# ORNL-Fusion/RAYS

Measured on AMD Instinct MI355X. Metric: ray-steps/sec (whole node), 64k-ray Solovev fan, higher is better.
Workload: dtype f64

## Files before the change

### rays_amd/csrc/rays_device_arith.inc

```
RAYS_DEV double sq(double x) { return x * x; }
RAYS_DEV double pow4(double x) { return ((x * x) * x) * x; }

constexpr int kEqUnitExp = 4;
constexpr int kEqMultiSpec = 8;
constexpr int kEqTol = 16;
constexpr int kEqNoTraj = 32;
constexpr int kEqDeposit = 64;
template <bool MULTI, int NS, int NV>
struct RayVec {
  static constexpr bool DAMP = MULTI || NV == 8 || NV == 13;
  static constexpr int NV0 = 7 + (DAMP ? 1 : 0) + (MULTI ? NS : 0);
  static constexpr bool GRAD = NV == NV0 + 5;
  static_assert(NV == NV0 || NV == NV0 + 5, "nv does not match the damping / gradient options");
};
template <bool UE, bool Y1>
RAYS_DEV double pow_u(double x, double y) {
  if (UE) return Y1 ? x : 1.0;
  if (y == 1.0) return x;
  if (y == 0.0) return 1.0;
  return libm::pow(x, y);
}

struct Recip {
  double d, rc;
// ... 535 lines not shown
    return;
  }
#endif
  const double* const grid = table == 0 ? P.a_rb_grid : (table == 1 ? P.a_ne_grid : (table == 2 ? P.a_te_grid : P.a_ti_grid));
  const double* const fspl = table == 0 ? P.a_rb_fspl : (table == 1 ? P.a_ne_fspl : (table == 2 ? P.a_te_fspl : P.a_ti_fspl));
  spl1_ax<const double*>(grid, fspl, n, P.a_axis[kAxRb + table], x, f, fp);
}

RAYS_DEV void spl1_tab_profiles(const DevParams& P, double psiN, double f[3], double fp[3]) {
  const int n[3] = {P.a_n_ne, P.a_n_te, P.a_n_ti};
#ifndef RAYS_HOST_EMUL
  if (P.a_lds_tab) {
    const eq_lds_ptr base = (eq_lds_ptr)(unsigned long long)P.a_lds_tab;
    const eq_lds_ptr grid[3] = {base + P.a_tab_off[2], base + P.a_tab_off[4], base + P.a_tab_off[6]};
    const eq_lds_ptr fspl[3] = {base + P.a_tab_off[3], base + P.a_tab_off[5], base + P.a_tab_off[7]};
    spl1_ax3<eq_lds_ptr>(grid, fspl, n, &P.a_axis[kAxNe], P.a_profiles_one_grid, psiN, f, fp);
    return;
  }
#endif
  const double* const grid[3] = {P.a_ne_grid, P.a_te_grid, P.a_ti_grid};
  const double* const fspl[3] = {P.a_ne_fspl, P.a_te_fspl, P.a_ti_fspl};
  spl1_ax3<const double*>(grid, fspl, n, &P.a_axis[kAxNe], P.a_profiles_one_grid, psiN, f, fp);
}

RAYS_DEV double eqlin_psi_at(const DevParams& P, int i, int j) {
  long long k = (long long)(i - 1) + (long long)(j - 1) * P.a_nr;
  const long long n = (long long)P.a_nr * P.a_nz;
  k = k < 0 ? 0 : (k >= n ? n - 1 : k);
  return P.a_psi_fspl[k];
}
RAYS_DEV double eqlin_getpsi(const DevParams& P, double R, double Z) {
  const double r1 = P.a_r_grid[0], z1 = P.a_z_grid[0];
  const Recip Rhr = make_recip(P.a_r_grid[1] - r1), Rhz = make_recip(P.a_z_grid[1] - z1);
  const int i = 1 + (int)div(R - r1, Rhr);
  const int j = 1 + (int)div(Z - z1, Rhz);
  const int ic = i < 1 ? 1 : (i > P.a_nr ? P.a_nr : i), jc = j < 1 ? 1 : (j > P.a_nz ? P.a_nz : j);
  const double x = div(R - P.a_r_grid[ic - 1], Rhr);
  const double y = div(Z - P.a_z_grid[jc - 1], Rhz);
  const double omx = 1. - x, omy = 1. - y;
  return ((eqlin_psi_at(P, i, j) * omx * omy + eqlin_psi_at(P, i + 1, j) * x * omy) + eqlin_psi_at(P, i, j + 1) * omx * y) +
         eqlin_psi_at(P, i + 1, j + 1) * x * y;
}
RAYS_DEV double eqlin_getrbphi(const DevParams& P, double R) {
  const double r1 = P.a_r_grid[0];
  const Recip Rhr = make_recip(P.a_r_grid[1] - r1);
  const int i = 1 + (int)div(R - r1, Rhr);
  const int ic = i < 1 ? 1 : (i > P.a_nr - 1 ? P.a_nr - 1 : i);
  const double x = div(R - P.a_r_grid[ic - 1], Rhr);
  return P.a_rb_fspl[ic - 1] * (1. - x) + P.a_rb_fspl[ic] * x;
}
RAYS_DEV void eqlin_psi_grad(const DevParams& P, double R, double Z, double& psi, double& PsiR, double& PsiZ) {
  const double dR = P.a_lin_dR, dZ = P.a_lin_dZ;
  psi = eqlin_getpsi(P, R, Z);
  PsiR = (eqlin_getpsi(P, R + dR, Z) - eqlin_getpsi(P, R - dR, Z)) / 2. / dR;
  PsiZ = (eqlin_getpsi(P, R, Z + dZ) - eqlin_getpsi(P, R, Z - dZ)) / 2. / dZ;
}
RAYS_DEV void eqlin_magnetics(const DevParams& P, double x, double y, double z, double r, const Recip& Rr, double bvec[3],
                              double gbt[3][3], double& psiN, double gradpsiN[3]) {
  const double dR = P.a_lin_dR, dZ = P.a_lin_dZ;
  double psi, PsiR, PsiZ;
  eqlin_psi_grad(P, r, z, psi, PsiR, PsiZ);
  const Recip Rr2 = recip_of_square(sq(r), Rr);
  const Recip RpsiB = const_recip(P.a_psiB, P.a_inv_psiB);
  const double br = div(-PsiZ, Rr);
  const double bz = div(PsiR, Rr);
  const double bphi = div(eqlin_getrbphi(P, r), Rr);
  const double gradpsi[3] = {x * bz, y * bz, -r * br};
  psiN = div(psi, RpsiB);
  gradpsiN[0] = div(gradpsi[0], RpsiB);
  gradpsiN[1] = div(gradpsi[1], RpsiB);
  gradpsiN[2] = div(gradpsi[2], RpsiB);
  const double PsiRZ = (((eqlin_getpsi(P, r + dR, z + dZ) - eqlin_getpsi(P, r - dR, z + dZ)) - eqlin_getpsi(P, r + dR, z - dZ)) +
                        eqlin_getpsi(P, r - dR, z - dZ)) / 4. / dR / dZ;
  const double PsiZZ = ((eqlin_getpsi(P, r, z + 2. * dZ) - 2. * psi) + eqlin_getpsi(P, r, z - 2. * dZ)) / dZ / dZ;
  const double PsiRR = ((eqlin_getpsi(P, r + 2. * dR, z) - 2. * psi) + eqlin_getpsi(P, r - 2. * dR, z)) / dR / dR;
  const double RBphiR = (eqlin_getrbphi(P, r + dR) - eqlin_getrbphi(P, r - dR)) / 2. / dR;
  const double br_r = div(br, Rr), bphi_r = div(bphi, Rr);
  const double dbrdr = -br_r - div(PsiRZ, Rr);
  const double dbrdz = div(-PsiZZ, Rr);
  const double dbzdr = div(-bz, Rr) + div(PsiRR, Rr);
  const double dbzdz = div(PsiRZ, Rr);
  const double dbphidr = div(RBphiR - bphi, Rr);
  bvec[0] = div(br * x, Rr) - div(bphi * y, Rr);
  bvec[1] = div(br * y, Rr) + div(bphi * x, Rr);
  bvec[2] = bz;
  const double x2 = sq(x), y2 = sq(y);
  gbt[0][0] = div(dbrdr * x2 + div(br * y2, Rr) + (-dbphidr + bphi_r) * x * y, Rr2);
  gbt[1][0] = div((dbrdr - br_r) * x * y - dbphidr * y2 - div(bphi * x2, Rr), Rr2);
  gbt[2][0] = div(dbrdz * x, Rr);
  gbt[0][1] = div((dbrdr - br_r) * x * y + dbphidr * x2 + div(bphi * y2, Rr), Rr2);
  gbt[1][1] = div(dbrdr * y2 + div(br * x2, Rr) + (dbphidr - bphi_r) * x * y, Rr2);
  gbt[2][1] = div(dbrdz * y, Rr);
  gbt[0][2] = div(dbzdr * x, Rr);
  gbt[1][2] = div(dbzdr * y, Rr);
  gbt[2][2] = dbzdz;
}

template <int NS, bool UE>
RAYS_DEV int axisym_fields(const DevParams& P, const double rvec[3], double bvec[3], double gbt[3][3],
                           double ns[NS], double gradns[NS][3], double ts[NS], double gradts[NS][3],
                           bool check_box) {
  constexpr double Tiny = 10.0e-14;
  int err = 0;
  const double x = rvec[0], y = rvec[1], z = rvec[2];
  Recip Rr;
  const double r = fsqrt_recip(x * x + y * y, Rr);
  if (r < P.a_box_rmin - Tiny || r > P.a_box_rmax + Tiny) err = RAYS_STOP_AXI_R_OUT_OF_BOX;
  if (z < P.a_box_zmin - Tiny || z > P.a_box_zmax + Tiny) err = RAYS_STOP_AXI_Z_OUT_OF_BOX;
  bool boxed = check_box && err != 0;
  double psiN, gpN[3];
  if (P.a_mag_model == RAYS_AXI_MAG_SOLOVEV) {
    int merr = 0;
    if (r < P.box_rmin || r > P.box_rmax) merr = RAYS_STOP_SOLMAG_R_OUT_OF_BOUNDS;
    if (z < P.box_zmin || z > P.box_zmax) merr = RAYS_STOP_SOLMAG_Z_OUT_OF_BOUNDS;
    if (check_box && !boxed && merr != 0) {
      boxed = true;
      err = merr;
    }
    solovev_magnetics(P, x, y, z, r, Rr, bvec, gbt, psiN, gpN);
  } else if (P.a_mag_model == RAYS_AXI_MAG_EQDSK_LIN) {
    eqlin_magnetics(P, x, y, z, r, Rr, bvec, gbt, psiN, gpN);
  } else {
    double f6[6], RBphi, RBphiR;
    spl2_fpp(P, r, z, f6);
    const double psi = f6[0], PsiR = f6[1], PsiZ = f6[2], PsiRR = f6[3], PsiRZ = f6[4], PsiZZ = f6[5];
    spl1_tab(P, 0, r, RBphi, RBphiR);
    const Recip Rr2 = recip_of_square(sq(r), Rr);
    const Recip RpsiB = const_recip(P.a_psiB, P.a_inv_psiB);
    const double br = div(PsiZ, Rr), bz = div(-PsiR, Rr), bphi = div(RBphi, Rr);
    const double gradpsi[3] = {-x * bz, -y * bz, r * br};
    psiN = div(psi, RpsiB);
    gpN[0] = div(gradpsi[0], RpsiB);
    gpN[1] = div(gradpsi[1], RpsiB);
    gpN[2] = div(gradpsi[2], RpsiB);
    const double br_r = div(br, Rr), bphi_r = div(bphi, Rr);
    const double dbrdr = -br_r + div(PsiRZ, Rr);
    const double dbrdz = div(PsiZZ, Rr);
    const double dbzdr = div(-bz, Rr) - div(PsiRR, Rr);
    const double dbzdz = div(-PsiRZ, Rr);
    const double dbphidr = div(RBphiR - bphi, Rr);
    bvec[0] = div(br * x, Rr) - div(bphi * y, Rr);
    bvec[1] = div(br * y, Rr) + div(bphi * x, Rr);
    bvec[2] = bz;
    const double x2 = sq(x), y2 = sq(y);
    gbt[0][0] = div(dbrdr * x2 + div(br * y2, Rr) + (-dbphidr + bphi_r) * x * y, Rr2);
    gbt[1][0] = div((dbrdr - br_r) * x * y - dbphidr * y2 - div(bphi * x2, Rr), Rr2);
    gbt[2][0] = div(dbrdz * x, Rr);
    gbt[0][1] = div((dbrdr - br_r) * x * y + dbphidr * x2 + div(bphi * y2, Rr), Rr2);
    gbt[1][1] = div(dbrdr * y2 + div(br * x2, Rr) + (dbphidr - bphi_r) * x * y, Rr2);
    gbt[2][1] = div(dbrdz * y, Rr);
    gbt[0][2] = div(dbzdr * x, Rr);
    gbt[1][2] = div(dbzdr * y, Rr);
    gbt[2][2] = dbzdz;
  }
  if (!boxed) err = 0;
  if (!boxed && psiN > P.a_psi_limit) err = RAYS_STOP_OUT_OF_PLASMA;

  bool t_spline = false;
#pragma unroll
  for (int is = 0; is < NS; is++) t_spline = t_spline || P.a_t_model[is] == RAYS_AXI_T_SPLINE;
  const bool batched = t_spline && P.a_n_model == RAYS_AXI_N_SPLINE && P.a_n_ne > 1 && P.a_n_te > 1 && P.a_n_ti > 1;
  double prof[3] = {0., 0., 0.}, dprof[3] = {0., 0., 0.};
  if (batched) spl1_tab_profiles(P, psiN, prof, dprof);

  if (P.a_n_model == RAYS_AXI_N_CONSTANT) {
#pragma unroll
    for (int is = 0; is < NS; is++) {
      ns[is] = P.n0s[is];
      gradns[is][0] = gradns[is][1] = gradns[is][2] = 0.;
    }
  } else {
    double dens = 0., dd_psi = 0.;
    if (P.a_n_model == RAYS_AXI_N_PARABOLIC) {
      parabolic_prof<UE>(psiN, P.a_d_scrape, P.a_an1, P.a_an2, dens, dd_psi);
    } else {
      {
        double d = prof[0], dp = dprof[0];
        if (!batched) spl1_tab(P, 1, psiN, d, dp);
        if (psiN <= 1.0) {
          dens = d;
          dd_psi = dp;
        }
      }
      if (dens < P.a_d_scrape) {
        dens = P.a_d_scrape;
        dd_psi = 0.;
      }
    }
#pragma unroll
    for (int is = 0; is < NS; is++) {
      ns[is] = P.n0s[is] * dens;
      const double c = P.n0s[is] * dd_psi;
      gradns[is][0] = c * gpN[0];
      gradns[is][1] = c * gpN[1];
      gradns[is][2] = c * gpN[2];
    }
  }
#pragma unroll
  for (int is = 0; is < NS; is++) {
    ts[is] = 0.;
    gradts[is][0] = gradts[is][1] = gradts[is][2] = 0.;
  }
#pragma unroll
  for (int is = 0; is < NS; is++) {
    const int m = P.a_t_model[is];
    if (m == RAYS_AXI_T_CONSTANT) {
      ts[is] = P.t0s[is];
#pragma unroll
      for (int j = 0; j < NS; j++) gradts[j][0] = gradts[j][1] = gradts[j][2] = 0.;
    } else if (m == RAYS_AXI_T_PARABOLIC) {
      double t_prof, dt_dpsi;
      parabolic_prof<UE>(psiN, P.a_T_scrape, P.a_at1[is], P.a_at2[is], t_prof, dt_dpsi);
      ts[is] = P.t0s[is] * t_prof;
      const double c = P.t0s[is] * dt_dpsi;
      gradts[is][0] = c * gpN[0];
      gradts[is][1] = c * gpN[1];
      gradts[is][2] = c * gpN[2];
    } else if (m == RAYS_AXI_T_SPLINE) {
      double Te = 0., dTe = 0., Ti = 0., dTi = 0.;
      {
        double te = prof[1], dte = dprof[1], ti = prof[2], dti = dprof[2];
        if (!batched) {
          spl1_tab(P, 2, psiN, te, dte);
          spl1_tab(P, 3, psiN, ti, dti);
        }
        if (psiN <= 1.0) {
          Te = te, dTe = dte, Ti = ti, dTi = dti;
        }
      }
      if (Te < P.a_T_scrape) { Te = P.a_T_scrape; dTe = 0.; }
      if (Ti < P.a_T_scrape) { Ti = P.a_T_scrape; dTi = 0.; }
      const double T = is == 0 ? Te : Ti, dT = is == 0 ? dTe : dTi;
      ts[is] = P.t0s[is] * T;
      const double c = P.t0s[is] * dT;
      gradts[is][0] = c * gpN[0];
      gradts[is][1] = c * gpN[1];
      gradts[is][2] = c * gpN[2];
    }
  }
  if (check_box && !boxed) {
    double mn = ns[0], mt = ts[0];
#pragma unroll
    for (int is = 1; is < NS; is++) {
      if (ns[is] < mn) mn = ns[is];
      if (ts[is] < mt) mt = ts[is];
    }
    if (mn < 0.) err = RAYS_STOP_NEGATIVE_DENS;
    if (mt < 0.) err = RAYS_STOP_NEGATIVE_TEMP;
  }
  return check_box ? err : 0;
}

template <int EQ, int NS, bool LEAN = false>
RAYS_DEV void equilibrium(const DevParams& P, const Recip& Romgrf, const Recip& Romgrf2,
                          const double rvec[3], EqPoint<NS>& eq, bool check_box) {
  double ns[NS], gradns[NS][3], ts[NS], gradts[NS][3];
  int err;
  constexpr int MODEL = EQ & 3;
  constexpr bool UE = (EQ & kEqUnitExp) != 0;
  if (MODEL == RAYS_EQ_SLAB)
    err = slab_fields<NS, UE>(P, rvec, eq.bvec, eq.gbt, ns, gradns, ts, gradts, check_box);
  else if (MODEL == RAYS_EQ_SOLOVEV)
    err = solovev_fields<NS, UE, LEAN>(P, rvec, eq.bvec, eq.gbt, ns, gradns, ts, gradts, check_box);
  else
    err = axisym_fields<NS, UE>(P, rvec, eq.bvec, eq.gbt, ns, gradns, ts, gradts, check_box);
  eq.err = err;
  Recip Rb;
  const double bmag = fsqrt_recip(sq(eq.bvec[0]) + sq(eq.bvec[1]) + sq(eq.bvec[2]), Rb);
  eq.bmag = bmag;
  eq.rbmag = Rb;
#pragma unroll
  for (int i = 0; i < 3; i++) eq.bunit[i] = div(eq.bvec[i], Rb);
#pragma unroll
  for (int i = 0; i < 3; i++)
    eq.gradbmag[i] = eq.gbt[i][0] * eq.bunit[0] + eq.gbt[i][1] * eq.bunit[1] + eq.gbt[i][2] * eq.bunit[2];
#pragma unroll
  for (int i = 0; i < 3; i++)
#pragma unroll
    for (int j = 0; j < 3; j++)
      eq.gradbunit[i][j] = div(eq.gbt[i][j] - eq.gradbmag[i] * eq.bunit[j], Rb);
#pragma unroll
  for (int is = 0; is < NS; is++) {
    eq.ns[is] = ns[is];
#pragma unroll
    for (int i = 0; i < 3; i++) eq.gradns[is][i] = gradns[is][i];
    const double omgc = div(P.qs[is] * bmag, const_recip(P.ms[is], P.inv_ms[is]));
    const double omgp2 = div(ns[is] * P.qs2[is], const_recip(P.eps0ms[is], P.inv_eps0ms[is]));
#if defined(RAYS_TOL_FLAVOUR) && !defined(RAYS_HOST_EMUL)
    eq.alpha[is] = ns[is] * P.alp_per_n[is];
    eq.gamma[is] = bmag * P.gam_per_b[is];
#else
    eq.alpha[is] = div(omgp2, Romgrf2);
    eq.gamma[is] = div(omgc, Romgrf);
#endif
    eq.omgc[is] = omgc;
    eq.omgp2[is] = omgp2;
    if (is == 0) eq.omgc0 = omgc;
  }
  eq.ts0 = ts[0];
#pragma unroll
  for (int i = 0; i < 3; i++) eq.gradts0[i] = gradts[0][i];
}

template <int NS>
RAYS_DEV void deriv_cold(const DevParams& P, const EqPoint<NS>& eq, const double nvec[3],
                         double dddx[3], double dddk[3], double& dddw) {
  const Recip Rk0 = const_recip(P.k0, P.inv_k0);
  double alpha[NS], gamma[NS];
#pragma unroll
  for (int is = 0; is < NS; is++) {
    alpha[is] = eq.alpha[is];
    gamma[is] = eq.gamma[is];
  }
  const double n3 = nvec[0] * eq.bunit[0] + nvec[1] * eq.bunit[1] + nvec[2] * eq.bunit[2];
  double np[3];
#pragma unroll
  for (int i = 0; i < 3; i++) np[i] = nvec[i] - n3 * eq.bunit[i];
#if defined(RAYS_TOL_FLAVOUR) && !defined(RAYS_HOST_EMUL)
  const double n1_2 = sq(np[0]) + sq(np[1]) + sq(np[2]);
#define RAYS_N1_SQ n1_2
#else
  const double n1 = fsqrt(sq(np[0]) + sq(np[1]) + sq(np[2]));
#define RAYS_N1_SQ sq(n1)
#endif
  double dn3dk[3], dn12dk[3], dn3dx[3], dn12dx[3];
#pragma unroll
  for (int i = 0; i < 3; i++) {
    dn3dk[i] = div(eq.bunit[i], Rk0);
    dn12dk[i] = P.two_over_k0 * np[i];
#if defined(RAYS_TOL_FLAVOUR) && !defined(RAYS_HOST_EMUL)
    dn3dx[i] = div((eq.gbt[i][0] * nvec[0] + eq.gbt[i][1] * nvec[1] + eq.gbt[i][2] * nvec[2]) - eq.gradbmag[i] * n3, eq.rbmag);
#else
    dn3dx[i] = eq.gradbunit[i][0] * nvec[0] + eq.gradbunit[i][1] * nvec[1] + eq.gradbunit[i][2] * nvec[2];
#endif
    dn12dx[i] = -2. * n3 * dn3dx[i];
  }
  double dadx[3][NS], dgdx[3][NS];
#pragma unroll
  for (int is = 0; is < NS; is++) {
    const Recip Rns = make_recip(eq.ns[is]);
#pragma unroll
    for (int i = 0; i < 3; i++) {
      dadx[i][is] = div(eq.alpha[is] * eq.gradns[is][i], Rns);
      dgdx[i][is] = div(gamma[is] * eq.gradbmag[i], eq.rbmag);
    }
  }
  const double dn3dw = div(-n3, const_recip(P.omgrf, P.inv_omgrf));
  const double dn12dw = P.m2_over_omgrf * RAYS_N1_SQ;
  double dadw[NS], dgdw[NS];
#pragma unroll
  for (int is = 0; is < NS; is++) {
    dadw[is] = P.m2_over_omgrf * alpha[is];
    dgdw[is] = P.m1_over_omgrf * gamma[is];
  }
  double sa = 0.;
#pragma unroll
  for (int is = 0; is < NS; is++) sa += alpha[is];
  const double p = 1. - sa;
  double t = 1.;
#pragma unroll
  for (int is = 0; is < NS; is++) t *= (1. - sq(gamma[is]));
  double dq1da[NS], dq2da[NS];
#pragma unroll
  for (int is1 = 0; is1 < NS; is1++) {
    dq1da[is1] = 1.;
    dq2da[is1] = 1.;
#pragma unroll
    for (int is = 0; is < NS; is++)
      if (is != is1) {
        dq1da[is1] = dq1da[is1] * (1. + gamma[is]);
        dq2da[is1] = dq2da[is1] * (1. - gamma[is]);
      }
  }
  double q1 = 0., q2 = 0., su = 0.;
#pragma unroll
  for (int is = 0; is < NS; is++) q1 += alpha[is] * dq1da[is];
#pragma unroll
  for (int is = 0; is < NS; is++) q2 += alpha[is] * dq2da[is];
#pragma unroll
  for (int is = 0; is < NS; is++) su += alpha[is] * dq1da[is] * dq2da[is];
  const double u = t - su;
  const double q = 2. * u - t + q1 * q2;
#if defined(RAYS_TOL_FLAVOUR) && !defined(RAYS_HOST_EMUL)
  const double n3_2 = sq(n3), n3_4 = sq(n3_2), n1_4 = sq(n1_2);
#else
  const double n3_2 = sq(n3), n3_4 = pow4(n3), n1_2 = sq(n1), n1_4 = pow4(n1);
#endif
#undef RAYS_N1_SQ
  double duda[NS], dqda[NS], ddda[NS];
#pragma unroll
  for (int is = 0; is < NS; is++) {
    duda[is] = -dq1da[is] * dq2da[is];
    dqda[is] = 2. * duda[is] + dq1da[is] * q2 + q1 * dq2da[is];
    ddda[is] = -t * n3_4 + (2. * (u - p * duda[is]) + (-t + duda[is]) * n1_2) * n3_2 - q +
               p * dqda[is] - (dqda[is] - u + p * duda[is]) * n1_2 + duda[is] * n1_4;
  }
  double gp[NS][NS], gm[NS][NS], gpm[NS][NS];
#pragma unroll
  for (int is1 = 0; is1 < NS; is1++)
#pragma unroll
    for (int is2 = 0; is2 < NS; is2++) {
      double a = 1., b = 1.;
#pragma unroll
      for (int is = 0; is < NS; is++)
        if (is != is1 && is != is2) {
          a = a * (1. + gamma[is]);
          b = b * (1. - gamma[is]);
        }
      gp[is1][is2] = a;
      gm[is1][is2] = b;
      gpm[is1][is2] = a * b;
    }
  double dtdg[NS], dudg[NS], dq1dg[NS], dq2dg[NS], dqdg[NS], dddg[NS];
#pragma unroll
  for (int is = 0; is < NS; is++) dtdg[is] = 2. * gamma[is] * duda[is];
#pragma unroll
  for (int is = 0; is < NS; is++) {
    double a = 0., b = 0., c = 0.;
#pragma unroll
    for (int j = 0; j < NS; j++) {
      a += alpha[j] * gpm[j][is];
      b += alpha[j] * gp[j][is];
      c += alpha[j] * gm[j][is];
    }
    dudg[is] = dtdg[is] + 2. * gamma[is] * (a + alpha[is] * duda[is]);
    dq1dg[is] = b - alpha[is] * dq1da[is];
    dq2dg[is] = -c + alpha[is] * dq2da[is];
    dqdg[is] = 2. * dudg[is] - dtdg[is] + dq1dg[is] * q2 + q1 * dq2dg[is];
    dddg[is] = dtdg[is] * p * n3_4 + (-2. * p * dudg[is] + (dtdg[is] * p + dudg[is]) * n1_2) * n3_2 +
               p * dqdg[is] - (dqdg[is] + p * dudg[is]) * n1_2 + dudg[is] * n1_4;
  }
  const double dddn3 = (4. * t * p * n3_2 + 2. * (-2. * p * u + (t * p + u) * n1_2)) * n3;
  const double dddn12 = (t * p + u) * n3_2 - (q + p * u) + 2. * u * n1_2;
#if defined(RAYS_TOL_FLAVOUR) && !defined(RAYS_HOST_EMUL)
  double wg = 0., wa = 0.;
#pragma unroll
  for (int is = 0; is < NS; is++) {
    wg += dddg[is] * gamma[is];
    wa += ddda[is] * alpha[is];
  }
  const double c3 = dddn3 - 2. * n3 * dddn12, twon12 = 2. * dddn12;
#pragma unroll
  for (int i = 0; i < 3; i++) {
    dddk[i] = P.inv_k0 * (dddn3 * eq.bunit[i] + twon12 * np[i]);
    double a = 0.;
#pragma unroll
    for (int is = 0; is < NS; is++) a += ddda[is] * dadx[i][is];
    dddx[i] = a + wg * (eq.gradbmag[i] * eq.rbmag.rc) + c3 * dn3dx[i];
  }
  dddw = P.m1_over_omgrf * (2. * wa + wg + dddn3 * n3 + twon12 * n1_2);
  (void)dn3dk; (void)dn12dk; (void)dn12dx; (void)dgdx; (void)dadw; (void)dgdw; (void)dn3dw; (void)dn12dw;
#else
#pragma unroll
  for (int i = 0; i < 3; i++) {
    dddk[i] = dddn3 * dn3dk[i] + dddn12 * dn12dk[i];
    double a = 0.;
#pragma unroll
    for (int is = 0; is < NS; is++) a += ddda[is] * dadx[i][is] + dddg[is] * dgdx[i][is];
    dddx[i] = a + dddn3 * dn3dx[i] + dddn12 * dn12dx[i];
  }
  double a = 0.;
#pragma unroll
  for (int is = 0; is < NS; is++) a += ddda[is] * dadw[is] + dddg[is] * dgdw[is];
  dddw = a + dddn3 * dn3dw + dddn12 * dn12dw;
#endif
}

template <int NS>
RAYS_DEV void eps_cold(const double alpha[NS], const double gamma[NS], double& e11, double& e33,
                       double& x12) {
  double s11 = 0., s33 = 0., s12 = 0.;
#pragma unroll
  for (int is = 0; is < NS; is++) {
    const double omg2 = 1. - sq(gamma[is]);
    s11 = s11 + fdiv(-alpha[is], omg2);
    s33 = s33 + (-alpha[is]);
    s12 = s12 + (-divdc3_real(alpha[is] * gamma[is], omg2));
  }
  e11 = s11 + 1.0;
  e33 = s33 + 1.0;
  x12 = s12;
}

RAYS_DEV double epsn_det(double e11, double e33, double x12, double n1, double n3, double nsq) {
  const double E11 = e11 + n1 * n1 - nsq;
  const double E22 = e11 + 0. * 0. - nsq;
  const double E33 = e33 + n3 * n3 - nsq;
  const double E13 = 0. + n1 * n3 - 0. * nsq;
  return E33 * (E11 * E22 - x12 * x12) - E13 * (E22 * E13);
}

struct DetermEps {
  double e11, e33, x12, pr;
};
template <int NS>
RAYS_DEV DetermEps determ_eps(const double alpha[NS], const double gamma[NS]) {
  DetermEps E;
  eps_cold<NS>(alpha, gamma, E.e11, E.e33, E.x12);
  double pr = 1.;
#pragma unroll
  for (int is = 0; is < NS; is++) pr *= (1. - sq(gamma[is]));
  E.pr = pr;
  return E;
}
RAYS_DEV double determ_k(const double bunit[3], const DetermEps& E, const double kvec[3], const Recip& Rk0) {
  const double k3 = kvec[0] * bunit[0] + kvec[1] * bunit[1] + kvec[2] * bunit[2];
  const double k1 = fsqrt(sq(kvec[0] - k3 * bunit[0]) + sq(kvec[1] - k3 * bunit[1]) + sq(kvec[2] - k3 * bunit[2]));
  const double n1 = div(k1, Rk0), n3 = div(k3, Rk0);
  const double nsq = sq(n1) + 0. + sq(n3);
  const double det = epsn_det(E.e11, E.e33, E.x12, n1, n3, nsq);
  return det * E.pr;
}
template <int NS>
RAYS_DEV double determ(const double bunit[3], const double alpha[NS], const double gamma[NS],
                       const double kvec[3], const Recip& Rk0) {
  return determ_k(bunit, determ_eps<NS>(alpha, gamma), kvec, Rk0);
}

template <int EQ, int NS>
RAYS_DEV void eq_for_determ(const DevParams& P, const Recip& Romgrf, const Recip& Romgrf2,
                            const double rvec[3], double bunit[3], double alpha[NS], double gamma[NS]) {
  EqPoint<NS> e;
  equilibrium<EQ, NS>(P, Romgrf, Romgrf2, rvec, e, false);
#pragma unroll
  for (int i = 0; i < 3; i++) bunit[i] = e.bunit[i];
#pragma unroll
  for (int is = 0; is < NS; is++) {
    alpha[is] = e.alpha[is];
    gamma[is] = e.gamma[is];
  }
}

template <int EQ, int NS>
RAYS_DEV void deriv_num(const DevParams& P, const EqPoint<NS>& eq0, const double rvec0[3],
                        const double kvec0[3], double dddx[3], double dddk[3], double& dddw) {
  double bu[3], al[NS], ga[NS];
  const Recip Ro = const_recip(P.omgrf, P.inv_omgrf), Ro2 = const_recip(P.omgrf2, P.inv_omgrf2);
  const Recip Rk0 = const_recip(P.k0, P.inv_k0);
#pragma unroll 1
  for (int i = 0; i < 3; i++) {
    double rp[3], rm[3];
#pragma unroll
    for (int c = 0; c < 3; c++) {
      rp[c] = (c == i) ? rvec0[c] + P.delta : rvec0[c];
      rm[c] = (c == i) ? rvec0[c] - P.delta : rvec0[c];
    }
    eq_for_determ<EQ, NS>(P, Ro, Ro2, rp, bu, al, ga);
    const double det_plus = determ<NS>(bu, al, ga, kvec0, Rk0);
    eq_for_determ<EQ, NS>(P, Ro, Ro2, rm, bu, al, ga);
    const double det_minus = determ<NS>(bu, al, ga, kvec0, Rk0);
    const double d = (det_plus - det_minus) / P.two_delta;
    if (i == 0) dddx[0] = d;
    if (i == 1) dddx[1] = d;
    if (i == 2) dddx[2] = d;
  }
  const DetermEps E0 = determ_eps<NS>(eq0.alpha, eq0.gamma);
#pragma unroll 1
  for (int i = 0; i < 3; i++) {
    const double ki = (i == 0) ? kvec0[0] : (i == 1) ? kvec0[1] : kvec0[2];
    const double change = fmax(P.delta, fabs(P.delta * ki)) / 2.;
    double kp[3], km[3];
#pragma unroll
    for (int c = 0; c < 3; c++) {
      kp[c] = (c == i) ? kvec0[c] + change : kvec0[c];
      km[c] = (c == i) ? kvec0[c] - change : kvec0[c];
    }
    const double det_plus = determ_k(eq0.bunit, E0, kp, Rk0);
    const double det_minus = determ_k(eq0.bunit, E0, km, Rk0);
    const double d = (det_plus - det_minus) / (2. * change);
    if (i == 0) dddk[0] = d;
    if (i == 1) dddk[1] = d;
    if (i == 2) dddk[2] = d;
  }
  (void)bu;
#pragma unroll
  for (int is = 0; is < NS; is++) {
    al[is] = div(eq0.omgp2[is], const_recip(P.omgrf2_p, P.inv_omgrf2_p));
    ga[is] = div(eq0.omgc[is], const_recip(P.omgrf_p, P.inv_omgrf_p));
  }
  const double det_plus = determ<NS>(eq0.bunit, al, ga, kvec0, const_recip(P.k0_p, P.inv_k0_p));
#pragma unroll
  for (int is = 0; is < NS; is++) {
    al[is] = div(eq0.omgp2[is], const_recip(P.omgrf2_m, P.inv_omgrf2_m));
    ga[is] = div(eq0.omgc[is], const_recip(P.omgrf_m, P.inv_omgrf_m));
  }
  const double det_minus = determ<NS>(eq0.bunit, al, ga, kvec0, const_recip(P.k0_m, P.inv_k0_m));
  dddw = (det_plus - det_minus) / P.omgrf0_delta;
}

RAYS_DEV double powi_rt(double a, int b) {
  const bool recip = b < 0;
  double r = 1.;
  while (true) {
    if (b & 1) r = r * a;
    b /= 2;
    if (b == 0) break;
    a = a * a;
  }
  return recip ? 1. / r : r;
}

struct Cplx {
  double re, im;
};
RAYS_DEV Cplx divdc3(Cplx x, Cplx y) {
  double c = y.re, d = y.im;
#if defined(RAYS_TOL_FLAVOUR) && !defined(RAYS_HOST_EMUL)
  {
    const Recip Rd = make_recip(c * c + d * d);
    return Cplx{div(x.re * c + x.im * d, Rd), div(x.im * c - x.re * d, Rd)};
  }
#endif
  const double m = fmax(fabs(c), fabs(d));
  int k = 0;
  if (m > 0.0 && m < __builtin_inf()) {
    k = ilogb(m);
    c = scalbn(c, -k);
    d = scalbn(d, -k);
  }
  const double denom = c * c + d * d;
  Cplx r;
  r.re = scalbn((x.re * c + x.im * d) / denom, -k);
  r.im = scalbn((x.im * c - x.re * d) / denom, -k);
  return r;
}

RAYS_DEV double zf_x(const DevParams& P, int i, const Recip& Rn) {
  RAYS_FP_AS_WRITTEN
  return P.zf_xmin + div((double)(i - 1) * (P.zf_xmax - P.zf_xmin), Rn);
}

RAYS_DEV Cplx zfun_real_arg_spline(const DevParams& P, double z) {
  RAYS_FP_AS_WRITTEN
  double re;
  if (fabs(z) <= 10.0) {
    const int nxm = P.zf_nx - 1;
    const Recip Rn = make_recip((double)nxm);
    const double x1 = zf_x(P, 1, Rn), xn = zf_x(P, P.zf_nx, Rn);
    const double t = 1 + fdiv(nxm * (z - x1), xn - x1);
    int i = (int)t;
    i = i < nxm ? i : nxm;
    i = i > 1 ? i : 1;
    if (z < zf_x(P, i, Rn)) i = i - 1;
    else if (z > zf_x(P, i + 1, Rn)) i = i + 1;
    i = i < 1 ? 1 : (i > nxm ? nxm : i);
    const double dx = z - zf_x(P, i, Rn);
    double f0, f1, f2, f3;
#ifndef RAYS_HOST_EMUL
    if (P.zf_lds) {
      const eq_lds_ptr f = (eq_lds_ptr)(unsigned long long)P.zf_lds + 4 * (i - 1);
      f0 = f[0]; f1 = f[1]; f2 = f[2]; f3 = f[3];
    } else
#endif
    {
      const double* f = P.zf_fspl + 4 * (long long)(i - 1);
      f0 = f[0]; f1 = f[1]; f2 = f[2]; f3 = f[3];
    }
    re = f0 + dx * (f1 + dx * (f2 + dx * f3));
  } else {
    const double A[6] = {1., 1. / 2., 3. / 4., 15. / 8., 105. / 16., 945. / 32.};
    const double z_inv = 1.0 / z;
    re = 0.;
    for (int i = 1; i <= 6; i++) re = re - powi_rt(z_inv, 2 * i - 1) * A[i - 1];
  }
  Cplx r;
  r.re = re;
  r.im = 1.7724538509055159 * libm::exp(-(z * z));
  return r;
}

template <int NS>
RAYS_DEV double damp_fund_ech(const DevParams& P, const EqPoint<NS>& eq, const double kvec[3],
                              const double vg[3]) {
  const double k0 = P.k0;
  const Recip Rk0 = const_recip(P.k0, P.inv_k0);
  const double nvec[3] = {div(kvec[0], Rk0), div(kvec[1], Rk0), div(kvec[2], Rk0)};
  const double k3 = kvec[0] * eq.bunit[0] + kvec[1] * eq.bunit[1] + kvec[2] * eq.bunit[2];
  const double k1 = fsqrt(sq(kvec[0] - k3 * eq.bunit[0]) + sq(kvec[1] - k3 * eq.bunit[1]) +
                         sq(kvec[2] - k3 * eq.bunit[2]));
  const double R3 = div(k3, Rk0), R1 = div(k1, Rk0);
  const double R1S = sq(R1), R3S = sq(R3), RS = R1S + R3S;
  const double B1 = eq.gamma[0], BETAE = sq(B1);
  if (R3 == 0.) return 0.;
  const double vth = fsqrt(fdiv(2. * eq.ts0, P.ms[0]));
  const double VT = fdiv(vth, P.clight);
  const double xi = fdiv(P.omgrf + eq.omgc0, k3 * vth);
  if (fabs(xi) > 5.) return 0.;
  Cplx zf;
  if (k3 > 0.) {
    zf = zfun_real_arg_spline(P, xi);
  } else {
    zf = zfun_real_arg_spline(P, -xi);
    zf.re = -zf.re;
    zf.im = -zf.im;
  }
  const double Pa = eq.alpha[0];
  const double Q = fdiv(Pa / 2., 1 - B1);
  const double L1 = (1. - Q) * RS * R1S + (1. - Pa) * RS * R3S - (1. - Q) * (1. - Pa) * (RS + R3S) -
                    (1 - 2. * Q) * R1S + (1 - 2 * Q) * (1 - Pa);
  const double L2 = -(fdiv(Pa, B1) * (RS * R1S - (1. - 2. * Q) * R1S)) +
                    fdiv(fdiv(Pa * Pa / 4., BETAE) * R1S, R3S) * (RS + R3S - 2. * (1. - 2. * Q));
  const double L5 = Pa * (RS * R3S - (1. - Q) * (RS + R3S) + (1. - 2. * Q));
  const double F = (1. - B1) * R3 * VT * (L1 + L2 + fdiv(fdiv(R1S / 2., R3), BETAE) * VT * xi * L5);
  const Cplx one = {1., 0.};
  const Cplx zinv = divdc3(one, zf);
  const double par_re = xi + zinv.re, par_im = 0. + zinv.im;
  const float dw_re = (float)(-(F * par_re - 0. * par_im));
  const float dw_im = (float)(-(0. * par_re + F * par_im));
  const double A = 1. - Pa - BETAE;
  const double B = -((1. - Pa) * A + sq(1. - Pa) - BETAE) + (A + (1. - Pa) * (1. - BETAE)) * R3S;
  const double DDNX2 = 2. * A * R1S + B;
  const double DDNZ = 2. * R3 * ((A + (1. - Pa) * (1. - BETAE)) * R1S + (1 - Pa) * (2. * (1. - BETAE) * R3S - 2. * A));
  const double nvg = fsqrt(sq(vg[0]) + sq(vg[1]) + sq(vg[2]));
  double dot = 0.;
#pragma unroll
  for (int i = 0; i < 3; i++) {
    const double ddn = DDNX2 * (2 * (nvec[i] - R3 * eq.bunit[i])) + DDNZ * eq.bunit[i];
    dot += ddn * fdiv(vg[i], nvg);
  }
  const Cplx num = {-(double)dw_re, -(double)dw_im};
  const Cplx den = {dot, 0.};
  const float delta_im = (float)divdc3(num, den).im;
  return k0 * (double)delta_im;
}

template <int NS, int NV, bool MULTI = false, bool LEAN = false>
RAYS_DEV int ray_equations(const DevParams& P, const EqPoint<NS>& eq, const double kvec[3], double v7,
                           const double dddx[3], const double dddk[3], double dddw, double dvds[NV]) {
  if (!(dddw != 0.)) return RAYS_STOP_INFINITE_VG_RHS;
  const Recip Rw = make_recip(dddw);
  double vg[3];
#pragma unroll
  for (int i = 0; i < 3; i++) vg[i] = div(-dddk[i], Rw);
  const double vg0 = fsqrt(sq(vg[0]) + sq(vg[1]) + sq(vg[2]));
  double dsd;
  if (!LEAN && P.ray_param == RAYS_PARAM_ARCL) {
    if (dddk[0] != 0. || dddk[1] != 0. || dddk[2] != 0.) {
      const double sgn = copysign(1.0, dddw);
      const Recip Rnk = make_recip(fsqrt(sq(dddk[0]) + sq(dddk[1]) + sq(dddk[2])));
#pragma unroll
      for (int i = 0; i < 3; i++) {
        dvds[i] = div(-sgn * dddk[i], Rnk);
        dvds[3 + i] = div(sgn * dddx[i], Rnk);
      }
      dsd = 1.;
    } else {
      return RAYS_STOP_RAY_STALLED;
    }
  } else {
#pragma unroll
    for (int i = 0; i < 3; i++) {
      dvds[i] = vg[i];
      dvds[3 + i] = div(dddx[i], Rw);
    }
    dsd = vg0;
  }
  dvds[6] = dsd;
  typedef RayVec<MULTI, NS, NV> L;
  constexpr bool DAMP = L::DAMP;
  constexpr int NV0 = L::NV0;
  if (DAMP) {
    const double ki = damp_fund_ech<NS>(P, eq, kvec, vg);
    dvds[7] = dsd * 2. * ki * (1. - v7);
    if (MULTI) {
#pragma unroll
      for (int is = 0; is < NS; is++) dvds[8 + is] = dsd * 2. * (is == 0 ? ki : 0.) * (1. - v7);
    }
  }
  if (L::GRAD) {
    const Recip Rvg0 = make_recip(vg0);
    double vu[3];
#pragma unroll
    for (int i = 0; i < 3; i++) vu[i] = div(vg[i], Rvg0);
#pragma unroll
    for (int j = 0; j < 3; j++)
      dvds[NV0 + j] = dsd * vu[0] * eq.gbt[0][j] + dsd * vu[1] * eq.gbt[1][j] + dsd * vu[2] * eq.gbt[2][j];
    dvds[NV0 + 3] = dsd * vu[0] * eq.gradns[0][0] + dsd * vu[1] * eq.gradns[0][1] + dsd * vu[2] * eq.gradns[0][2];
    dvds[NV0 + 4] = dsd * vu[0] * eq.gradts0[0] + dsd * vu[1] * eq.gradts0[1] + dsd * vu[2] * eq.gradts0[2];
  }
  return 0;
}

template <int EQ, int NS, int DERIV, int NV>
RAYS_DEV int eqn_ray(const DevParams& P, const double v[NV], double dvds[NV]) {
  const double rvec[3] = {v[0], v[1], v[2]}, kvec[3] = {v[3], v[4], v[5]};
  EqPoint<NS> eq;
  equilibrium<EQ, NS>(P, const_recip(P.omgrf, P.inv_omgrf), const_recip(P.omgrf2, P.inv_omgrf2), rvec, eq, true);
  if (eq.err) return eq.err;
  double dddx[3], dddk[3], dddw;
  if (DERIV == RAYS_DERIV_COLD) {
    const Recip Rk0 = const_recip(P.k0, P.inv_k0);
    const double nvec[3] = {div(kvec[0], Rk0), div(kvec[1], Rk0), div(kvec[2], Rk0)};
    deriv_cold<NS>(P, eq, nvec, dddx, dddk, dddw);
  } else {
    deriv_num<EQ, NS>(P, eq, rvec, kvec, dddx, dddk, dddw);
  }
  constexpr bool MULTI = (EQ & kEqMultiSpec) != 0;
  return ray_equations<NS, NV, MULTI>(P, eq, kvec, v[RayVec<MULTI, NS, NV>::DAMP ? 7 : 0], dddx, dddk, dddw, dvds);
}

template <int EQ, int NS, int DERIV, int NV, bool LEAN = false>
RAYS_DEV void rhs_eval(const DevParams& P, const double v[NV], bool do_check, double& resid,
                       int& cs_flag, bool& cs_stop, int& code, double f[NV], double* cond = nullptr) {
  const double rvec[3] = {v[0], v[1], v[2]}, kvec[3] = {v[3], v[4], v[5]};
  EqPoint<NS> eq;
  equilibrium<EQ, NS, LEAN>(P, const_recip(P.omgrf, P.inv_omgrf), const_recip(P.omgrf2, P.inv_omgrf2), rvec, eq, true);
  const Recip Rk0 = const_recip(P.k0, P.inv_k0);
  const double nvec[3] = {div(kvec[0], Rk0), div(kvec[1], Rk0), div(kvec[2], Rk0)};
  cs_flag = 0;
  cs_stop = false;
  resid = 0.;
  if (do_check) {
    cs_flag = eq.err;
    const double k3 = kvec[0] * eq.bunit[0] + kvec[1] * eq.bunit[1] + kvec[2] * eq.bunit[2];
    const double k1 = fsqrt(sq(kvec[0] - k3 * eq.bunit[0]) + sq(kvec[1] - k3 * eq.bunit[1]) +
                           sq(kvec[2] - k3 * eq.bunit[2]));
    const double n1 = div(k1, Rk0), n3 = div(k3, Rk0);
    const double nsq = sq(n1) + 0. + sq(n3);
    double e11, e33, x12;
    eps_cold<NS>(eq.alpha, eq.gamma, e11, e33, x12);
    const double det = epsn_det(e11, e33, x12, n1, n3, nsq);
    const double N11 = fabs(e11) + fabs(n1 * n1), N22 = fabs(e11) + fabs(0. * 0.);
    const double N33 = fabs(e33) + fabs(n3 * n3), N12 = fabs(x12) + fabs(n1 * 0.);
    const double N13 = 0. + fabs(n1 * n3), N23 = 0. + fabs(0. * n3);
    const double den = N33 * (N11 * N22) + N33 * (N12 * N12) + N23 * (N11 * N23) + N23 * (N12 * N13) +
                       N13 * (N12 * N23) + N13 * (N22 * N13);
    resid = divdc3_real(fabs(det), den);
    if (resid > P.resid_limit) {
      cs_stop = true;
      cs_flag = RAYS_STOP_DISP_RESIDUAL;
    }
  }
  double dddx[3], dddk[3], dddw;
  if (DERIV == RAYS_DERIV_COLD || do_check) {
    deriv_cold<NS>(P, eq, nvec, dddx, dddk, dddw);
    if (do_check && !(fabs(dddw) > 2.2250738585072014e-308)) {
      cs_stop = true;
      cs_flag = RAYS_STOP_INFINITE_VG_CHECK;
    }
  }
  constexpr bool MULTI = (EQ & kEqMultiSpec) != 0;
  constexpr bool DAMP = RayVec<MULTI, NS, NV>::DAMP;
  if (do_check && DAMP) {
    if (v[DAMP ? 7 : 0] > P.total_damping_limit) {
      cs_stop = true;
      cs_flag = RAYS_STOP_TOTAL_ABSORPTION;
    }
  }
  if (DERIV == RAYS_DERIV_NUM) deriv_num<EQ, NS>(P, eq, rvec, kvec, dddx, dddk, dddw);
  const int rc = ray_equations<NS, NV, MULTI, LEAN>(P, eq, kvec, v[DAMP ? 7 : 0], dddx, dddk, dddw, f);
  code = eq.err ? eq.err : rc;
  if (cond) *cond = dddw;
}

template <int EQ, int NS, int DERIV, int NV>
RAYS_DEV int rk4_step_as_reference(const DevParams& P, const double v[NV], double dsl, double w[NV]) {
  const Recip R6 = const_recip(6.0, 1.0 / 6.0);
  double acc[NV], x[NV];
#pragma unroll
  for (int i = 0; i < NV; i++) {
    acc[i] = 0.;
    x[i] = v[i];
  }
  int stop = 0;
#pragma unroll 1
  for (int j = 0; j < 4; j++) {
    double f[NV], resid;
    int code, cs_flag;
    bool cs_stop;
    rhs_eval<EQ, NS, DERIV, NV>(P, x, false, resid, cs_flag, cs_stop, code, f);
    if (code != 0 && stop == 0) stop = code;
    const double wt = (j == 1 || j == 2) ? 2.0 : 1.0;
    const double half = j < 2 ? 0.5 : 1.0;
#pragma unroll
    for (int i = 0; i < NV; i++) {
      acc[i] = j == 0 ? f[i] : acc[i] + wt * f[i];
      x[i] = j < 3 ? v[i] + dsl * f[i] * half : v[i] + div(dsl * acc[i], R6);
    }
  }
#pragma unroll
  for (int i = 0; i < NV; i++) w[i] = x[i];
  return stop;
}

template <int EQ, int NS, int NV>
RAYS_DEV void initialize_ode_vector(const DevParams& P, const double* __restrict__ r0,
                                    const double* __restrict__ n0, double v[NV]) {
#pragma unroll
  for (int i = 0; i < 3; i++) {
    v[i] = r0[i];
    v[3 + i] = P.k0 * n0[i];
  }
  v[6] = 0.;
  typedef RayVec<(EQ & kEqMultiSpec) != 0, NS, NV> L;
  constexpr int NV0 = L::NV0;
#pragma unroll
  for (int i = 7; i < NV0; i++) v[i] = 0.;
  if (L::GRAD) {
    EqPoint<NS> eq;
    const double rvec[3] = {v[0], v[1], v[2]};
    equilibrium<EQ, NS>(P, const_recip(P.omgrf, P.inv_omgrf), const_recip(P.omgrf2, P.inv_omgrf2), rvec, eq, false);
    v[NV0] = eq.bvec[0];
    v[NV0 + 1] = eq.bvec[1];
    v[NV0 + 2] = eq.bvec[2];
    v[NV0 + 3] = eq.ns[0];
    v[NV0 + 4] = eq.ts0;
  }
}
```

Baseline: 7.345 billion.

## Factor cold dispersion derivatives into shared adjoint coefficients and reuse projections in residual check

After: 8.101 billion (median of 6 runs). +10.3%, better.

```diff
diff --git a/rays_amd/csrc/rays_cold_adjoint.inc b/rays_amd/csrc/rays_cold_adjoint.inc
--- /dev/null
+++ b/rays_amd/csrc/rays_cold_adjoint.inc
@@ -0,0 +1,18 @@
+template <int NS>
+RAYS_DEV void cold_adjoint(double p, double t, double u, double q, double n1_2, double n3_2, const double duda[NS],
+                           const double dqda[NS], const double dtdg[NS], const double dudg[NS], const double dqdg[NS],
+                           double ddda[NS], double dddg[NS]) {
+  const double n3_4 = n3_2 * n3_2, n1_4 = n1_2 * n1_2;
+  const double a1 = n1_2 * n3_2;
+  const double m = n3_4 + a1;
+  const double h = 2. * n3_2 + n1_2;
+  const double D_t = p * m;
+  const double D_p = t * m + q - u * h;
+  const double D_u = a1 + n1_4 - p * h;
+  const double D_q = p - n1_2;
+#pragma unroll
+  for (int is = 0; is < NS; is++) {
+    ddda[is] = D_u * duda[is] + D_q * dqda[is] - D_p;
+    dddg[is] = D_t * dtdg[is] + D_u * dudg[is] + D_q * dqdg[is];
+  }
+}
diff --git a/rays_amd/csrc/rays_device_arith.inc b/rays_amd/csrc/rays_device_arith.inc
--- a/rays_amd/csrc/rays_device_arith.inc
+++ b/rays_amd/csrc/rays_device_arith.inc
@@ -861,9 +861,17 @@
   for (int i = 0; i < 3; i++) eq.gradts0[i] = gradts[0][i];
 }
 
+#if defined(RAYS_TOL_FLAVOUR) && !defined(RAYS_HOST_EMUL)
+#include "rays_cold_adjoint.inc"
+#endif
+
 template <int NS>
 RAYS_DEV void deriv_cold(const DevParams& P, const EqPoint<NS>& eq, const double nvec[3],
-                         double dddx[3], double dddk[3], double& dddw) {
+                         double dddx[3], double dddk[3], double& dddw
+#if defined(RAYS_TOL_FLAVOUR) && !defined(RAYS_HOST_EMUL)
+                         , double* idx = nullptr
+#endif
+                         ) {
   const Recip Rk0 = const_recip(P.k0, P.inv_k0);
   double alpha[NS], gamma[NS];
 #pragma unroll
@@ -882,16 +890,19 @@
   const double n1 = fsqrt(sq(np[0]) + sq(np[1]) + sq(np[2]));
 #define RAYS_N1_SQ sq(n1)
 #endif
+#if defined(RAYS_TOL_FLAVOUR) && !defined(RAYS_HOST_EMUL)
+  (void)Rk0;
+  if (idx) {
+    idx[0] = n3;
+    idx[1] = n1_2;
+  }
+#else
   double dn3dk[3], dn12dk[3], dn3dx[3], dn12dx[3];
 #pragma unroll
   for (int i = 0; i < 3; i++) {
     dn3dk[i] = div(eq.bunit[i], Rk0);
     dn12dk[i] = P.two_over_k0 * np[i];
-#if defined(RAYS_TOL_FLAVOUR) && !defined(RAYS_HOST_EMUL)
-    dn3dx[i] = div((eq.gbt[i][0] * nvec[0] + eq.gbt[i][1] * nvec[1] + eq.gbt[i][2] * nvec[2]) - eq.gradbmag[i] * n3, eq.rbmag);
-#else
     dn3dx[i] = eq.gradbunit[i][0] * nvec[0] + eq.gradbunit[i][1] * nvec[1] + eq.gradbunit[i][2] * nvec[2];
-#endif
     dn12dx[i] = -2. * n3 * dn3dx[i];
   }
   double dadx[3][NS], dgdx[3][NS];
@@ -912,6 +923,7 @@
     dadw[is] = P.m2_over_omgrf * alpha[is];
     dgdw[is] = P.m1_over_omgrf * gamma[is];
   }
+#endif
   double sa = 0.;
 #pragma unroll
   for (int is = 0; is < NS; is++) sa += alpha[is];
@@ -941,7 +953,7 @@
   const double u = t - su;
   const double q = 2. * u - t + q1 * q2;
 #if defined(RAYS_TOL_FLAVOUR) && !defined(RAYS_HOST_EMUL)
-  const double n3_2 = sq(n3), n3_4 = sq(n3_2), n1_4 = sq(n1_2);
+  const double n3_2 = sq(n3);
 #else
   const double n3_2 = sq(n3), n3_4 = pow4(n3), n1_2 = sq(n1), n1_4 = pow4(n1);
 #endif
@@ -951,8 +963,11 @@
   for (int is = 0; is < NS; is++) {
     duda[is] = -dq1da[is] * dq2da[is];
     dqda[is] = 2. * duda[is] + dq1da[is] * q2 + q1 * dq2da[is];
+#if defined(RAYS_TOL_FLAVOUR) && !defined(RAYS_HOST_EMUL)
+#else
     ddda[is] = -t * n3_4 + (2. * (u - p * duda[is]) + (-t + duda[is]) * n1_2) * n3_2 - q +
                p * dqda[is] - (dqda[is] - u + p * duda[is]) * n1_2 + duda[is] * n1_4;
+#endif
   }
   double gp[NS][NS], gm[NS][NS], gpm[NS][NS];
 #pragma unroll
@@ -986,29 +1001,37 @@
     dq1dg[is] = b - alpha[is] * dq1da[is];
     dq2dg[is] = -c + alpha[is] * dq2da[is];
     dqdg[is] = 2. * dudg[is] - dtdg[is] + dq1dg[is] * q2 + q1 * dq2dg[is];
+#if defined(RAYS_TOL_FLAVOUR) && !defined(RAYS_HOST_EMUL)
+  }
+  cold_adjoint<NS>(p, t, u, q, n1_2, n3_2, duda, dqda, dtdg, dudg, dqdg, ddda, dddg);
+#else
     dddg[is] = dtdg[is] * p * n3_4 + (-2. * p * dudg[is] + (dtdg[is] * p + dudg[is]) * n1_2) * n3_2 +
                p * dqdg[is] - (dqdg[is] + p * dudg[is]) * n1_2 + dudg[is] * n1_4;
   }
+#endif
   const double dddn3 = (4. * t * p * n3_2 + 2. * (-2. * p * u + (t * p + u) * n1_2)) * n3;
   const double dddn12 = (t * p + u) * n3_2 - (q + p * u) + 2. * u * n1_2;
 #if defined(RAYS_TOL_FLAVOUR) && !defined(RAYS_HOST_EMUL)
-  double wg = 0., wa = 0.;
+  double wg = 0., wa = 0., e[NS];
 #pragma unroll
   for (int is = 0; is < NS; is++) {
     wg += dddg[is] * gamma[is];
     wa += ddda[is] * alpha[is];
+    const Recip Rns = make_recip(eq.ns[is]);
+    e[is] = ddda[is] * (alpha[is] * Rns.rc);
   }
   const double c3 = dddn3 - 2. * n3 * dddn12, twon12 = 2. * dddn12;
+  const double cg = wg - c3 * n3;
 #pragma unroll
   for (int i = 0; i < 3; i++) {
     dddk[i] = P.inv_k0 * (dddn3 * eq.bunit[i] + twon12 * np[i]);
+    const double gn = eq.gbt[i][0] * nvec[0] + eq.gbt[i][1] * nvec[1] + eq.gbt[i][2] * nvec[2];
     double a = 0.;
 #pragma unroll
-    for (int is = 0; is < NS; is++) a += ddda[is] * dadx[i][is];
-    dddx[i] = a + wg * (eq.gradbmag[i] * eq.rbmag.rc) + c3 * dn3dx[i];
+    for (int is = 0; is < NS; is++) a += e[is] * eq.gradns[is][i];
+    dddx[i] = a + eq.rbmag.rc * (c3 * gn + cg * eq.gradbmag[i]);
   }
   dddw = P.m1_over_omgrf * (2. * wa + wg + dddn3 * n3 + twon12 * n1_2);
-  (void)dn3dk; (void)dn12dk; (void)dn12dx; (void)dgdx; (void)dadw; (void)dgdw; (void)dn3dw; (void)dn12dw;
 #else
 #pragma unroll
   for (int i = 0; i < 3; i++) {
@@ -1369,6 +1392,30 @@
   cs_flag = 0;
   cs_stop = false;
   resid = 0.;
+#if defined(RAYS_TOL_FLAVOUR) && !defined(RAYS_HOST_EMUL)
+  static_assert(DERIV == RAYS_DERIV_COLD, "the tolerance flavour exists for the cold derivatives only");
+  double dddx[3], dddk[3], dddw, idx[2];
+  deriv_cold<NS>(P, eq, nvec, dddx, dddk, dddw, idx);
+  if (do_check) {
+    cs_flag = eq.err;
+    const double n3_2 = sq(idx[0]), n1_2 = idx[1], x13 = n1_2 * n3_2;
+    double e11, e33, x12;
+    eps_cold<NS>(eq.alpha, eq.gamma, e11, e33, x12);
+    const double E11 = e11 - n3_2, E22 = E11 - n1_2, E33 = e33 - n1_2;
+    const double det = E33 * (E11 * E22 - x12 * x12) - E22 * x13;
+    const double N11 = fabs(e11) + n1_2, N22 = fabs(e11), N33 = fabs(e33) + n3_2, N12 = fabs(x12);
+    const double den = N33 * (N11 * N22) + N33 * (N12 * N12) + N22 * x13;
+    resid = divdc3_real(fabs(det), den);
+    if (resid > P.resid_limit) {
+      cs_stop = true;
+      cs_flag = RAYS_STOP_DISP_RESIDUAL;
+    }
+    if (!(fabs(dddw) > 2.2250738585072014e-308)) {
+      cs_stop = true;
+      cs_flag = RAYS_STOP_INFINITE_VG_CHECK;
+    }
+  }
+#else
   if (do_check) {
     cs_flag = eq.err;
     const double k3 = kvec[0] * eq.bunit[0] + kvec[1] * eq.bunit[1] + kvec[2] * eq.bunit[2];
@@ -1398,6 +1445,7 @@
       cs_flag = RAYS_STOP_INFINITE_VG_CHECK;
     }
   }
+#endif
   constexpr bool MULTI = (EQ & kEqMultiSpec) != 0;
   constexpr bool DAMP = RayVec<MULTI, NS, NV>::DAMP;
   if (do_check && DAMP) {
```
